# victorca25/traiNNer

Measured on AMD Instinct MI355X. Metric: HR images/sec (G+D step), ESRGAN x4 128->512, higher is better.
Workload: dtype f32 (bf16x3)

## Files before the change

### trainner_amd/csrc/conv_epilogue.h

```cpp
#pragma once
#include "conv_body.h"

namespace {

template <int MODE, int TW, int NT, int MT, bool COH, int DEPTH = 1, bool NOISE = true, int BIAS_STEP = 1, class PixFn>
__device__ __forceinline__ void conv_epilogue_dpp_map(const ConvK a, f32x16 (&acc)[MT][NT], const int cb, const int n, const int ty0,
                                                      const int tx0, const int par, const int li, const int half,
                                                      const __amdgpu_buffer_rsrc_t y_rs, PixFn &&pixfn) {
    constexpr bool DG2 = (MODE == TNR_DGRAD_4x4_S2);
    constexpr int NC = NT * 32;
    const int py = par >> 1, px = par & 1;
    TNR_STAMP(2);
#ifdef TNR_PRIO_EPI
    __builtin_amdgcn_s_setprio(TNR_PRIO_EPI);
#endif
    const int qa = li >> 2, qb = li & 3;
    const bool b0 = (qb & 1) != 0, b1 = (qb & 2) != 0;
    auto quad_transpose = [&](float &v0, float &v1, float &v2, float &v3) {
        auto xchg = [&](float &x, float &y, bool sel, int which) {
            const float send = sel ? x : y;
            const int r_ = which == 1 ? __builtin_amdgcn_mov_dpp(__builtin_bit_cast(int, send), 0xB1, 0xF, 0xF, true)
                                      : __builtin_amdgcn_mov_dpp(__builtin_bit_cast(int, send), 0x4E, 0xF, 0xF, true);
            const float recv = __builtin_bit_cast(float, r_);
            x = sel ? recv : x;
            y = sel ? y : recv;
        };
        xchg(v0, v1, b0, 1);
        xchg(v2, v3, b0, 1);
        xchg(v0, v2, b1, 2);
        xchg(v1, v3, b1, 2);
    };
    TNR_STAMP(5);
    TNR_STAMP(6);
    TNR_STAMP(7);
#ifdef TNR_ABL_NOMASK
    const bool has_r1 = a.r1 != nullptr, has_r2 = a.r2 != nullptr, has_m = false;
#else
    const bool has_r1 = a.r1 != nullptr, has_r2 = a.r2 != nullptr, has_m = a.m != nullptr;
#endif
    const bool has_noise = NOISE && a.noise_pos != 0;
    const bool all_full = (a.Cout & 3) == 0;
    const float ns = a.act == TNR_ACT_LRELU ? a.slope : (a.act == TNR_ACT_RELU ? 0.f : 1.f);
    int co_n[NT];
    bool co_ok[NT];
    f32x4 bv[NT];
    float b1f[NT], msf[NT];
    bool use_r1[NT], use_m[NT];
#pragma unroll
    for (int nn = 0; nn < NT; ++nn) {
        const int co = cb * NC + nn * 32 + qa * 4;
        co_n[nn] = co;
        co_ok[nn] = co < a.Cout;
        bv[nn] = f32x4{0.f, 0.f, 0.f, 0.f};
        if (a.bias != nullptr && co_ok[nn]) {
            if constexpr (BIAS_STEP != 1) {
#pragma unroll
                for (int k = 0; k < 4; ++k)
                    if (co + k < a.Cout) bv[nn][k] = a.bias[(co + k) * BIAS_STEP];
            } else if (co + 4 <= a.Cout) {
                bv[nn] = *reinterpret_cast<const f32x4 *>(a.bias + co);
            } else {
#pragma unroll
                for (int k = 0; k < 4; ++k)
                    if (co + k < a.Cout) bv[nn][k] = a.bias[co + k];
            }
        }
        use_r1[nn] = has_r1 && co < a.r1_ch;
        use_m[nn] = has_m && co >= a.m_lo && co < a.m_hi;
        b1f[nn] = use_r1[nn] ? a.beta1 : 0.f;
        msf[nn] = use_m[nn] ? a.m_slope : 1.f;
    }
    constexpr int UNITS = MT * 4;
    constexpr int AHEAD = DEPTH < UNITS ? DEPTH : UNITS, SETS = AHEAD + 1 < UNITS ? AHEAD + 1 : UNITS;
    bool ok[SETS];
    size_t pixi[SETS];
    f32x4 q1[SETS][NT], q2[SETS][NT], qm[SETS][NT];
    auto prep = [&](int u, int set) {
        const int mi = u >> 2, q = u & 3;
        int rr, cc;
        pixfn(mi, 8 * q + 4 * half + qb, rr, cc);
        const int sy = ty0 + rr, sx = tx0 + cc;
        ok[set] = sy < a.th_space && sx < a.tw_space;
        const int oy = DG2 ? 2 * sy + py : sy;
        const int ox = DG2 ? 2 * sx + px : sx;
        const size_t pix = ((size_t)n * a.Ho + oy) * a.Wo + ox;
        pixi[set] = pix;
        const f32x4 zero = {0.f, 0.f, 0.f, 0.f}, one = {1.f, 1.f, 1.f, 1.f};
#pragma unroll
        for (int nn = 0; nn < NT; ++nn) {
            const bool okc = ok[set] && co_ok[nn];
            if (has_r1) {
// ... 6 lines not shown
            }
            if (has_m) {
                qm[set][nn] = one;
                if (okc && use_m[nn]) qm[set][nn] = *reinterpret_cast<const f32x4 *>(a.m + pix * a.m_ct + a.m_co + co_n[nn]);
            }
        }
    };
    auto finish = [&](int u, int set) {
        const int mi = u >> 2, q = u & 3;
#pragma unroll
        for (int nn = 0; nn < NT; ++nn) {
            float v0 = acc[mi][nn][4 * q + 0], v1 = acc[mi][nn][4 * q + 1], v2 = acc[mi][nn][4 * q + 2], v3 = acc[mi][nn][4 * q + 3];
            quad_transpose(v0, v1, v2, v3);
            f32x4 v = f32x4{v0, v1, v2, v3} + bv[nn];
#pragma unroll
            for (int e = 0; e < 4; ++e) v[e] = __builtin_fmaf(ns, __builtin_fminf(v[e], 0.f), __builtin_fmaxf(v[e], 0.f)) * a.alpha;
            if (has_r1) v += b1f[nn] * q1[set][nn];
            if (has_noise) {
                const f32x4 nm = tnr_gauss_mult4(((unsigned)pixi[set] + a.noise_pix0) * (unsigned)(a.Cout >> 2) + (unsigned)(co_n[nn] >> 2),
                                                 a.noise_k0, a.noise_k1, a.noise_sigma);
                if (a.noise_pos == 1) v *= nm;
                if (has_r2) v = v * a.alpha2 + q2[set][nn];
                if (a.noise_pos != 1) v *= nm;
            } else if (has_r2) {
                v = v * a.alpha2 + q2[set][nn];
            }
            if (has_m) {
#pragma unroll
                for (int e = 0; e < 4; ++e) v[e] *= (qm[set][nn][e] > 0.f ? 1.f : msf[nn]);
            }
            if (!(ok[set] && co_ok[nn])) continue;
            const int co = co_n[nn];
#ifdef TNR_ABL_NOEPISTORE
            if (v[0] == 1.2345e30f) a.y[0] = v[1] + v[2] + v[3];
            continue;
#endif
            if (COH) {
                __builtin_amdgcn_raw_buffer_store_b128(__builtin_bit_cast(tnr_u32x4, v), y_rs,
                                                       (int)((unsigned)(pixi[set] * a.y_ct + a.y_co + co) * 4u), 0, TNR_COH_STORE_AUX);
            } else {
                float *yp = a.y + pixi[set] * a.y_ct + a.y_co + co;
                if (all_full) {
                    *reinterpret_cast<f32x4 *>(yp) = v;
                } else {
#pragma unroll
                    for (int e = 0; e < 4; ++e)
                        if (co + e < a.Cout) yp[e] = v[e];
                }
            }
        }
    };
#pragma unroll
    for (int u = 0; u < AHEAD; ++u) prep(u, u % SETS);
#pragma unroll
    for (int u = 0; u < UNITS; ++u) {
        if (u + AHEAD < UNITS) prep(u + AHEAD, (u + AHEAD) % SETS);
        finish(u, u % SETS);
    }
}

template <int MODE, int TW, int NT, int MT, bool COH, int DEPTH = 1, bool NOISE = true, int BIAS_STEP = 1>
__device__ __forceinline__ void conv_epilogue_dpp(const ConvK a, f32x16 (&acc)[MT][NT], const int cb, const int n, const int ty0,
                                                  const int tx0, const int par, const int wave, const int li, const int half,
                                                  const __amdgpu_buffer_rsrc_t y_rs) {
    conv_epilogue_dpp_map<MODE, TW, NT, MT, COH, DEPTH, NOISE, BIAS_STEP>(a, acc, cb, n, ty0, tx0, par, li, half, y_rs,
                                                                [&](int mi, int row, int &rr, int &cc) __attribute__((always_inline)) {
                                                                    const int p = (wave * MT + mi) * 32 + row;
                                                                    rr = p / TW;
                                                                    cc = p - rr * TW;
                                                                });
}

}
```

### trainner_amd/csrc/conv_sweep.hip

```cpp
#include <stddef.h>
#include <string.h>
#include <type_traits>
#include <utility>
#include "conv_body.h"
#include "conv_epilogue.h"
#include "conv_handoff.h"

namespace {

constexpr int SW_TH = 8, SW_TW = 32, SW_HT = SW_TH + 2, SW_WT = SW_TW + 2;
constexpr int SW_ROW = TNR_X3_ROW;
constexpr int SW_A_ROWS = SW_HT * SW_WT;
constexpr int SW_A_ALLOC_ROWS = 384;
constexpr int SW_A_FLOATS = SW_A_ALLOC_ROWS * SW_ROW;
constexpr int SW_UNIT_FLOATS = 32 * SW_ROW;
constexpr int SW_SLOT_UNITS = 9;
constexpr int SW_SLOT_FLOATS = SW_SLOT_UNITS * SW_UNIT_FLOATS;
constexpr int SW_RING = 3;
constexpr size_t SW_LDS_BYTES = (size_t)(2 * SW_A_FLOATS + SW_RING * SW_SLOT_FLOATS) * sizeof(float);
constexpr int SW_NPASS = 9, SW_NSTAGE = 5, SW_NTILE = 6;
constexpr int SW_A_IT = (SW_A_ROWS * 4 + 511) / 512;
constexpr int SW_B_PIECES = (SW_SLOT_UNITS * 3 + 7) / 8;
static_assert(SW_LDS_BYTES <= 160 * 1024, "one sweep workgroup per CU");

// ... 1083 lines not shown
        src = a.wp + (((size_t)par * 4 + tap) * a.KoutP + cb * 64 + j * 32 + r) * a.KinP + 16 * ck + 8 * h;
    } else {
        const int ck = rest % a.nck;
        rest /= a.nck;
        const int pp = rest & 3, cb = rest >> 2;
        src = a.wp + ((size_t)tap * a.KoutP + cb * 64 + j * 32 + r) * (4 * a.KinP) + pp * a.KinP + 16 * ck + 8 * h;
    }
    const f32x4 q0 = *reinterpret_cast<const f32x4 *>(src), q1 = *reinterpret_cast<const f32x4 *>(src + 4);
    tnr_bf16x8 pl[3];
    tnr_split_bf16x3(q0, q1, pl);
    float *dst = a.out + (size_t)unit * SW_UNIT_FLOATS + (h * 32 + r) * 4;
#pragma unroll
    for (int k = 0; k < 3; ++k) *reinterpret_cast<tnr_bf16x8 *>(dst + k * 256) = pl[k];
}

template <bool AMP, class Item, class BFetch>
__device__ __forceinline__ void tap4_chunk(f32x16 (&acc)[2][2], const float *sa, const int (&aaddr)[2][4], Item &&item_step,
                                           tnr_bf16x8 (&fbr)[S2_RING][3], BFetch &&b_fetch) {
    constexpr int TA[6] = {0, 2, 1, 0, 1, 0}, TB[6] = {2, 0, 1, 1, 0, 0};
    tnr_bf16x8 fa[2][2][3];
    auto read_a = [&](auto tc, int m, int sp) __attribute__((always_inline)) {
        constexpr int t = decltype(tc)::value;
        fa[t & 1][m][sp] = *reinterpret_cast<const tnr_bf16x8 *>(sa + aaddr[m][t] + 8 * sp);
    };
#pragma unroll
    for (int k = 0; k < (AMP ? 2 : 6); ++k) read_a(std::integral_constant<int, 0>{}, AMP ? k : k / 3, AMP ? 0 : k % 3);
    sw_static_for<0, S2_NU>([&](auto uc) __attribute__((always_inline)) {
        constexpr int u = decltype(uc)::value, t = u >> 1, jj = u & 1;
        constexpr bool NEXT_TAP = jj == 1 && t + 1 < S2_TAPS;
        constexpr int ITEM = u - (S2_NU - 6);
        __builtin_amdgcn_sched_barrier(0);
        if constexpr (AMP) {
            sw_static_for<0, 2>([&](auto mc) __attribute__((always_inline)) {
                constexpr int m = decltype(mc)::value;
                acc[m][jj] = __builtin_amdgcn_mfma_f32_32x32x16_bf16(fa[t & 1][m][0], fbr[u % S2_RING][0], acc[m][jj], 0, 0, 0);
                if constexpr (m == 0) b_fetch(std::integral_constant<int, (u + 3) % S2_RING>{}, 0);
                if constexpr (NEXT_TAP) read_a(std::integral_constant<int, (t + 1 < S2_TAPS ? t + 1 : t)>{}, m, 0);
                if constexpr (m == 1 && ITEM >= 0) item_step(std::integral_constant<int, (ITEM >= 0 ? ITEM : 0)>{}, std::integral_constant<int, -1>{});
                __builtin_amdgcn_sched_barrier(0);
            });
        } else {
            sw_static_for<0, 12>([&](auto ic) __attribute__((always_inline)) {
                constexpr int i = decltype(ic)::value, p = i / 2, m = i % 2;
                acc[m][jj] = __builtin_amdgcn_mfma_f32_32x32x16_bf16(fa[t & 1][m][TA[p]], fbr[u % S2_RING][TB[p]], acc[m][jj], 0, 0, 0);
                if constexpr (i < 3) b_fetch(std::integral_constant<int, (u + 3) % S2_RING>{}, i);
                if constexpr (NEXT_TAP && i >= 3 && i < 9) read_a(std::integral_constant<int, (t + 1 < S2_TAPS ? t + 1 : t)>{}, (i - 3) / 3, (i - 3) % 3);
                if constexpr (ITEM >= 0 && i >= 4 && i < 9) item_step(std::integral_constant<int, (ITEM >= 0 ? ITEM : 0)>{}, std::integral_constant<int, (i >= 4 && i < 9 ? i - 4 : 0)>{});
                __builtin_amdgcn_sched_barrier(0);
            });
        }
    });
}

template <int MODE, bool AMP>
__global__ void __launch_bounds__(256, 2) conv_s2_d4_kernel(const S2K c) {
    constexpr bool DG = MODE == TNR_DGRAD_4x4_S2;
    constexpr int HT = DG ? SW_HT : SW_TH + 1, WT = DG ? SW_WT : SW_TW + 1, ROWS = HT * WT;
    constexpr int A_IT = (ROWS * 4 + 255) / 256;
    static_assert(A_IT <= 6 && A_IT * 256 <= SW_A_ALLOC_ROWS * 4, "staging plan");
    extern __shared__ __attribute__((aligned(16))) float smem[];
    float *s_a = smem;
    const int tid = threadIdx.x;
    const int wave = __builtin_amdgcn_readfirstlane(tid >> 6), lane = tid & 63, li = lane & 31, half = lane >> 5;
    const ConvK &a = c.a;
    const __amdgpu_buffer_rsrc_t x_rs =
        __builtin_amdgcn_make_buffer_rsrc(const_cast<float *>(a.x), 0, (int)((unsigned)a.N * a.H * a.W * a.x_ct * 4u), 0x00020000);
    const __amdgpu_buffer_rsrc_t w_rs = __builtin_amdgcn_make_buffer_rsrc(const_cast<float *>(c.wq), 0, c.wq_bytes, 0x00020000);
    const __amdgpu_buffer_rsrc_t y_rs =
        __builtin_amdgcn_make_buffer_rsrc(a.y, 0, (int)((unsigned)a.N * a.Ho * a.Wo * a.y_ct * 4u), 0x00020000);
    const int nchunks = DG ? c.nck : 4 * c.nck;

    for (int tile = blockIdx.x; tile < c.tiles; tile += gridDim.x) {
        int rest = tile;
        const int cb = rest % c.ncb;
        rest /= c.ncb;
        int par = 0;
        if constexpr (DG) {
            par = rest & 3;
            rest >>= 2;
        }
        const int tx = rest % c.tiles_x;
        rest /= c.tiles_x;
        const int ty = rest % c.tiles_y, n = rest / c.tiles_y;
        const int ty0 = ty * SW_TH, tx0 = tx * SW_TW;
        const int py = par >> 1, px = par & 1;
        int aaddr[2][4];
#pragma unroll
        for (int m = 0; m < 2; ++m)
#pragma unroll
            for (int t = 0; t < 4; ++t) {
                const int pos_y = DG ? 1 + py - (t >> 1) : (t >> 1), pos_x = DG ? 1 + px - (t & 1) : (t & 1);
                const int pp = (2 * wave + m + pos_y) * WT + li + pos_x;
                aaddr[m][t] = pp * SW_ROW + 4 * (half ^ ((pp >> TNR_X3_SWZ) & 1));
            }
        int in_off[A_IT], a_dst[A_IT];
        auto plan = [&](int pp) __attribute__((always_inline)) {
#pragma unroll
            for (int it = 0; it < A_IT; ++it) {
                const int i = tid + it * 256, row = i >> 2, q = i & 3;
                const int hr = row / WT, hc = row - hr * WT;
                const int Y = DG ? ty0 + hr - 1 : 2 * (ty0 + hr) - 1 + (pp >> 1), X = DG ? tx0 + hc - 1 : 2 * (tx0 + hc) - 1 + (pp & 1);
                const bool in = (row < ROWS) & (Y >= 0) & (Y < a.H) & (X >= 0) & (X < a.W);
                in_off[it] = in ? (((n * a.H + Y) * a.W + X) * a.x_ct + a.x_co + q * 4) : -1;
                a_dst[it] = row * SW_ROW + 4 * ((q >> 1) ^ ((row >> TNR_X3_SWZ) & 1)) + 2 * (q & 1);
            }
        };
        plan(0);
// ... 34 lines not shown
        for (int m = 0; m < 2; ++m)
#pragma unroll
            for (int j = 0; j < 2; ++j)
#pragma unroll
                for (int r = 0; r < 16; ++r) acc[m][j][r] = 0.f;

        a_load(0, true);
        __syncthreads();
        tnr_bf16x8 fbr[S2_RING][3];
        int bq = (DG ? (par * c.ncb + cb) * c.nck : cb * 4 * c.nck) * S2_NU;
        auto b_fetch = [&](auto rc, int sp) __attribute__((always_inline)) {
            constexpr int r = decltype(rc)::value;
            if constexpr (AMP) {
                fbr[r][0] = __builtin_bit_cast(tnr_bf16x8, __builtin_amdgcn_raw_buffer_load_b128(w_rs, lane * 16, bq * 3072, 0));
                ++bq;
            } else {
                fbr[r][sp] = __builtin_bit_cast(tnr_bf16x8, __builtin_amdgcn_raw_buffer_load_b128(w_rs, lane * 16, (bq * 3 + sp) * 1024, 0));
                if (sp == 2) ++bq;
            }
        };
        sw_static_for<0, 3>([&](auto rc) __attribute__((always_inline)) {
#pragma unroll
            for (int sp = 0; sp < (AMP ? 1 : 3); ++sp) b_fetch(rc, sp);
        });
        sw_static_for<0, 6>([&](auto ic) __attribute__((always_inline)) {
            if constexpr (AMP) item_step_buf(ic, std::integral_constant<int, -1>{}, 0);
            else sw_static_for<0, 5>([&](auto kc) __attribute__((always_inline)) { item_step_buf(ic, kc, 0); });
        });
        bool has_next = false;
        int e = 0;
        auto item_step = [&](auto ic, auto kc) __attribute__((always_inline)) {
            if (has_next) item_step_buf(ic, kc, (e + 1) & 1);
        };
#pragma unroll 1
        for (int ck = 0; ck < nchunks; ++ck) {
            asm volatile("s_waitcnt lgkmcnt(0)\n\ts_barrier" ::: "memory");
            has_next = ck + 1 < nchunks;
            int ch_next = 16 * (ck + 1);
            if constexpr (!DG) {
                const int nx = ck + 1, ppn = nx / c.nck;
                ch_next = 16 * (nx - ppn * c.nck);
                if (has_next && ppn != ck / c.nck) plan(ppn);
            }
            a_load(ch_next, has_next);
            tap4_chunk<AMP>(acc, s_a + (e & 1) * SW_A_FLOATS, aaddr, item_step, fbr, b_fetch);
            ++e;
        }
        f32x16 t2[2][2];
#pragma unroll
        for (int m = 0; m < 2; ++m) {
            t2[m][0] = acc[m][0];
            t2[m][1] = acc[m][1];
        }
        conv_epilogue_dpp<MODE, SW_TW, 2, 2, false, 1>(a, t2, cb, n, ty0, tx0, par, wave, li, half, y_rs);
    }
}

bool s2_ok(const tnr_conv_desc *d) {
    if (d->mode != TNR_CONV_4x4_S2 && d->mode != TNR_DGRAD_4x4_S2) return false;
    const bool dg = d->mode == TNR_DGRAD_4x4_S2;
    const int tw = dg ? d->W : d->Wo, th = dg ? d->H : d->Ho;
    return (d->mma == TNR_MMA_BF16X3 || d->mma == TNR_MMA_BF16) && d->pad_mode == 0 && d->shuffle == 0 && (d->Cout % 64) == 0 && d->KoutP == d->Cout &&
           d->Cin == d->KinP && (d->Cin % 16) == 0 && d->Cin >= 32 && tw >= 32 && th >= 8 &&
           (dg ? (d->Ho == 2 * d->H && d->Wo == 2 * d->W) : (d->H == 2 * d->Ho && d->W == 2 * d->Wo)) &&
           buffers_addressable(*d) &&
           (int64_t)(d->Cout / 64) * (d->Cin / 16) * 4 * S2_NU * SW_UNIT_FLOATS * (int64_t)sizeof(float) < (1LL << 31);
}

bool d4_ok(const tnr_conv_desc *d) {
    if (d->shuffle != 0 && !(d->shuffle == 2 && (d->Cout % 256) == 0 && d->r1.ptr == nullptr && d->r2.ptr == nullptr && d->m.ptr == nullptr &&
                             d->noise_pos == 0 && d->pad_mode == 0 && (d->y.ctot % 4) == 0 &&
                             (int64_t)d->N * d->H * d->W * 4 * d->y.ctot < (1LL << 30)))
        return false;
    return d->mode == TNR_CONV_3x3 && (d->mma == TNR_MMA_BF16X3 || d->mma == TNR_MMA_BF16) && (d->pad_mode == 0 || (d->pad_mode == 1 && d->H >= 2 && d->W >= 2)) &&
           (d->Cout % 64) == 0 && d->KoutP == d->Cout &&
           d->Cin == d->KinP && (d->Cin % 16) == 0 && d->Cin >= 32 && d->Ho == d->H && d->Wo == d->W && d->W >= 32 && d->H >= 8 &&
           buffers_addressable(*d) &&
           (int64_t)(d->Cout / 64) * (d->Cin / 16) * 18 * SW_UNIT_FLOATS * (int64_t)sizeof(float) < (1LL << 31);
}

bool sweep_pattern(const tnr_conv_desc *st, int n, const char **why) {
    auto no = [&](const char *w) { if (why) *why = w; return false; };
    if (st == nullptr || (n != SW_NSTAGE && n != SW4_NSTAGE)) return no("not 5 (or 4) stages");
    if (n == SW4_NSTAGE && st[0].mma != TNR_MMA_BF16X3) return no("the four-stage form exists in bf16x3 only");
    const tnr_conv_desc &d0 = st[0];
    if (d0.Cin < 32 || (d0.Cin % 16) != 0) return no("block input channels must be a multiple of 16, >= 32");
    for (int i = 0; i < n; ++i) {
        const tnr_conv_desc &d = st[i];
        if (d.mode != TNR_CONV_3x3 || (d.mma != TNR_MMA_BF16X3 && d.mma != TNR_MMA_BF16) || d.mma != d0.mma || d.pad_mode != 0)
            return no("stage is not a zero-padded 3x3 in bf16x3 (or all stages with bf16 operands)");
        if (d.N != d0.N || d.H != d0.H || d.W != d0.W || d.Ho != d0.H || d.Wo != d0.W) return no("pixel grids differ");
        if (d.x.ptr != d0.x.ptr || d.x.ctot != d0.x.ctot || d.x.coff != d0.x.coff) return no("stages read different buffers");
        if (d.Cin != d0.Cin + 32 * i || d.KinP != d.Cin) return no("input channels do not grow by 32 per stage");
        if (d.Cout != (i < 4 ? 32 : 64) || d.KoutP != d.Cout) return no("output channels are not 32, 32, 32, 32, 64");
        if (i < 4 && (d.y.ptr != d0.x.ptr || d.y.ctot != d0.x.ctot || d.y.coff != d0.x.coff + d.Cin)) return no("stage output is not the next channel group");
        if (!views_aligned(d)) return no("x / y / r1 / r2 / mask views must be 4-channel aligned");
        if (d.noise_pos < 0 || d.noise_pos > 2 || (i < 4 && d.noise_pos != 0)) return no("the noise multiplier belongs to the last stage");
        if (!buffers_addressable(d)) return no("buffer above 4 GiB");
        if (!d.x.ptr || !d.y.ptr || !d.wp) return no("null pointer");
    }
    const tnr_conv_desc &dl = st[n - 1];
    if (n == SW_NSTAGE && dl.y.ptr == d0.x.ptr && dl.y.coff < d0.x.coff + dl.Cin && dl.y.coff + dl.Cout > d0.x.coff) return no("last stage overwrites its own input");
    return true;
}

int sweep_form() {
    static const int form = [] {
// ... 120 lines not shown
        k.tiles_x = c.tiles_x; k.tiles_y = c.tiles_y; k.ncb = d->KoutP / 32;
    }
    const int per_round = (cus / c.tpi) * c.tpi;
    const int grid = c.tiles < per_round ? c.tiles : per_round;
    const int form = sweep_form();
    if (n == SW4_NSTAGE) {
        TNR_REQUIRE(form == 5, "conv_sweep: four stages run in the direct four-wave form only");
        hipLaunchKernelGGL((conv_sweep4_kernel<true, false, SwPlan4>), dim3((unsigned)grid), dim3(256), S4D_LDS_BYTES, (hipStream_t)stream, c);
        return tnr_check_launch("conv_sweep");
    }
    if (stages[0].mma == TNR_MMA_BF16) {
        TNR_REQUIRE(form == 5, "conv_sweep: bf16 operands (use_amp) run in the direct four-wave form only");
        hipLaunchKernelGGL((conv_sweep4_kernel<true, true>), dim3((unsigned)grid), dim3(256), S4D_LDS_BYTES, (hipStream_t)stream, c);
        return tnr_check_launch("conv_sweep");
    }
    if (form == 8) hipLaunchKernelGGL(conv_sweep_kernel, dim3((unsigned)grid), dim3(512), SW_LDS_BYTES, (hipStream_t)stream, c);
    else if (form == 4) hipLaunchKernelGGL(conv_sweep4_kernel<false>, dim3((unsigned)grid), dim3(256), SW_LDS_BYTES, (hipStream_t)stream, c);
    else hipLaunchKernelGGL(conv_sweep4_kernel<true>, dim3((unsigned)grid), dim3(256), S4D_LDS_BYTES, (hipStream_t)stream, c);
    return tnr_check_launch("conv_sweep");
}

extern "C" int64_t tnr_conv_wq_bytes(const tnr_conv_desc *d) {
    if (d != nullptr && s2_ok(d)) return (int64_t)(d->Cout / 64) * (d->Cin / 16) * 4 * S2_NU * SW_UNIT_FLOATS * (int64_t)sizeof(float);
    if (d == nullptr || !d4_ok(d)) return 0;
    return (int64_t)(d->Cout / 64) * (d->Cin / 16) * 18 * SW_UNIT_FLOATS * (int64_t)sizeof(float);
}

extern "C" int tnr_conv_wq_pack(const tnr_conv_desc *d, void *image, int64_t image_bytes, void *stream) {
    if (d != nullptr && image != nullptr && d->wp != nullptr && s2_ok(d)) {
        S2PackK a;
        a.wp = d->wp; a.KinP = d->KinP; a.KoutP = d->KoutP; a.nck = d->Cin / 16; a.ncb = d->Cout / 64;
        a.dgrad = d->mode == TNR_DGRAD_4x4_S2;
        a.units = a.ncb * 4 * a.nck * S2_NU;
        TNR_REQUIRE((int64_t)a.units * SW_UNIT_FLOATS * (int64_t)sizeof(float) <= image_bytes, "conv_wq_pack: image buffer too small");
        a.out = static_cast<float *>(image);
        hipLaunchKernelGGL(s2_pack_kernel, dim3((unsigned)tnr_cdiv(a.units * 64, 256)), dim3(256), 0, (hipStream_t)stream, a);
        return tnr_check_launch("conv_wq_pack (four-tap form)");
    }
    TNR_REQUIRE(d != nullptr && image != nullptr && d->wp != nullptr && d4_ok(d), "conv_wq_pack: the launch cannot use a pre-split weight stream");
    D4PackK a;
    a.wp = d->wp; a.KinP = d->KinP; a.KoutP = d->KoutP; a.nck = d->Cin / 16; a.ncb = d->Cout / 64;
    a.units = a.ncb * a.nck * 18;
    a.shuffle = d->shuffle;
    TNR_REQUIRE((int64_t)a.units * SW_UNIT_FLOATS * (int64_t)sizeof(float) <= image_bytes, "conv_wq_pack: image buffer too small");
    a.out = static_cast<float *>(image);
    hipLaunchKernelGGL(d4_pack_kernel, dim3((unsigned)tnr_cdiv(a.units * 64, 256)), dim3(256), 0, (hipStream_t)stream, a);
    return tnr_check_launch("conv_wq_pack");
}

int tnr_launch_conv_s2_d4(const tnr_conv_desc *d, void *stream) {
    if (!s2_ok(d) || d->wq == nullptr || d->wq_bytes < tnr_conv_wq_bytes(d) || d->noise_pos != 0) return 1;
    static int cus = 0;
    if (const int rc = tnr_kernel_setup(&cus, "conv_s2_d4", {{conv_s2_d4_kernel<TNR_CONV_4x4_S2, false>, S4D_LDS_BYTES}, {conv_s2_d4_kernel<TNR_CONV_4x4_S2, true>, S4D_LDS_BYTES},
                                                             {conv_s2_d4_kernel<TNR_DGRAD_4x4_S2, false>, S4D_LDS_BYTES}, {conv_s2_d4_kernel<TNR_DGRAD_4x4_S2, true>, S4D_LDS_BYTES}}))
        return rc;
    const bool dg = d->mode == TNR_DGRAD_4x4_S2;
    S2K c;
    if (!stream_k_from_desc(c, *d, tnr_conv_wq_bytes(d), SW_TW, SW_TH, dg ? 4 : 1)) return 1;
    const unsigned grid = (unsigned)(c.tiles < 2 * cus ? c.tiles : 2 * cus);
    const bool amp = d->mma == TNR_MMA_BF16;
    if (dg) {
        if (amp) hipLaunchKernelGGL((conv_s2_d4_kernel<TNR_DGRAD_4x4_S2, true>), dim3(grid), dim3(256), S4D_LDS_BYTES, (hipStream_t)stream, c);
        else hipLaunchKernelGGL((conv_s2_d4_kernel<TNR_DGRAD_4x4_S2, false>), dim3(grid), dim3(256), S4D_LDS_BYTES, (hipStream_t)stream, c);
    } else {
        if (amp) hipLaunchKernelGGL((conv_s2_d4_kernel<TNR_CONV_4x4_S2, true>), dim3(grid), dim3(256), S4D_LDS_BYTES, (hipStream_t)stream, c);
        else hipLaunchKernelGGL((conv_s2_d4_kernel<TNR_CONV_4x4_S2, false>), dim3(grid), dim3(256), S4D_LDS_BYTES, (hipStream_t)stream, c);
    }
    return tnr_check_launch("conv_s2_d4");
}

int tnr_launch_conv3x3_d4(const tnr_conv_desc *d, void *stream) {
    if (!d4_ok(d) || d->wq == nullptr || d->wq_bytes < tnr_conv_wq_bytes(d) || d->noise_pos < 0 || d->noise_pos > 2) return 1;
    static int occ = [] { const char *e = getenv("TNR_D4_OCC"); return e ? atoi(e) : 2; }();
    static int cus = 0;
    if (const int rc = tnr_kernel_setup(&cus, "conv3x3_d4", {{conv3x3_d4_kernel<1>, S4D_LDS_BYTES}, {conv3x3_d4_kernel<2>, S4D_LDS_BYTES}, {conv3x3_d4_kernel<2, true>, S4D_LDS_BYTES},
                                                             {conv3x3_d4_kernel<2, false, true>, S4D_LDS_BYTES}, {conv3x3_d4_kernel<2, true, true>, S4D_LDS_BYTES}}))
        return rc;
    D4K c;
    if (!stream_k_from_desc(c, *d, tnr_conv_wq_bytes(d), SW_TW, SW_TH, 1)) return 1;
    const int slots = cus * (occ == 1 ? 1 : 2);
    const int grid = c.tiles < slots ? c.tiles : slots;
    if (d->shuffle == 2) {
        const unsigned g2 = (unsigned)(c.tiles < 2 * cus ? c.tiles : 2 * cus);
        if (d->mma == TNR_MMA_BF16) hipLaunchKernelGGL((conv3x3_d4_kernel<2, true, true>), dim3(g2), dim3(256), S4D_LDS_BYTES, (hipStream_t)stream, c);
        else hipLaunchKernelGGL((conv3x3_d4_kernel<2, false, true>), dim3(g2), dim3(256), S4D_LDS_BYTES, (hipStream_t)stream, c);
        return tnr_check_launch("conv3x3_d4 (pixel-shuffle store)");
    }
    if (d->mma == TNR_MMA_BF16) hipLaunchKernelGGL((conv3x3_d4_kernel<2, true>), dim3((unsigned)(c.tiles < 2 * cus ? c.tiles : 2 * cus)), dim3(256), S4D_LDS_BYTES, (hipStream_t)stream, c);
    else if (occ == 1) hipLaunchKernelGGL(conv3x3_d4_kernel<1>, dim3((unsigned)grid), dim3(256), S4D_LDS_BYTES, (hipStream_t)stream, c);
    else hipLaunchKernelGGL(conv3x3_d4_kernel<2>, dim3((unsigned)grid), dim3(256), S4D_LDS_BYTES, (hipStream_t)stream, c);
    return tnr_check_launch("conv3x3_d4");
}
```

### trainner_amd/csrc/conv_wino.hip

```cpp
#include <stddef.h>
#include <stdlib.h>
#include <type_traits>
#include <utility>
#include "conv_body.h"
#include "conv_epilogue.h"

namespace {

constexpr int WN_T = 16;
constexpr int WN_PT = WN_T / 2;
constexpr int WN_NP = WN_PT * WN_PT;
constexpr int WN_RAW_W = WN_T + 2;
constexpr int WN_RAW_PIX = WN_RAW_W * WN_RAW_W;
constexpr int WN_RAW_STRIDE = 24;
constexpr int WN_RAW_FLOATS = WN_RAW_PIX * WN_RAW_STRIDE;
constexpr int WN_ROW = TNR_X3_ROW;
constexpr int WN_VH_ROWS = 8 * WN_NP;
constexpr int WN_VH_FLOATS = WN_VH_ROWS * WN_ROW;
constexpr size_t WN_LDS_BYTES = (size_t)(2 * WN_VH_FLOATS + 2 * WN_RAW_FLOATS) * sizeof(float);
constexpr int WN_UNIT_FLOATS = 32 * WN_ROW;
constexpr int WN_STAGE_ITEMS = WN_RAW_PIX * 4;
constexpr int WN_STAGE_IT = (WN_STAGE_ITEMS / 2 + 255) / 256;
static_assert(WN_LDS_BYTES <= 160 * 1024, "one Winograd workgroup per CU");
static_assert(8 * 4 * 16 * 64 * sizeof(float) <= WN_LDS_BYTES, "the inverse transform's exchange fits the LDS");
// ... 14 lines not shown
struct WinoK {
    ConvK a;
    const float *wq;
    int wq_bytes;
    int nck;
    int tiles_x, tiles_y, ncb, tiles;
};

struct WinoPackK {
    const float *wp;
    int KinP, KoutP, nck, ncb, units;
    float *out;
};

__global__ void __launch_bounds__(256) wino_pack_kernel(const WinoPackK a) {
    const int g = blockIdx.x * 256 + threadIdx.x;
    const int unit = g >> 6, r = (g >> 1) & 31, oh = g & 1;
    if (unit >= a.units) return;
    const int j = unit & 3;
    int rest = unit >> 2;
    const int ck = rest % a.nck;
    rest /= a.nck;
    const int i = rest & 3, nt = (rest >> 2) & 1, cb = rest >> 3;
    const int co = cb * 64 + nt * 32 + r;
    const double G[4][3] = {{1.0, 0.0, 0.0}, {0.5, 0.5, 0.5}, {0.5, -0.5, 0.5}, {0.0, 0.0, 1.0}};
    f32x4 q[2];
#pragma unroll
    for (int e = 0; e < 8; ++e) {
        const int ch = 16 * ck + 8 * oh + e;
        double u = 0.0;
#pragma unroll
        for (int ky = 0; ky < 3; ++ky)
#pragma unroll
            for (int kx = 0; kx < 3; ++kx)
                u += G[i][ky] * G[j][kx] * (double)a.wp[((size_t)(ky * 3 + kx) * a.KoutP + co) * a.KinP + ch];
        q[e >> 2][e & 3] = (float)u;
    }
    tnr_bf16x8 pl[3];
    tnr_split_bf16x3(q[0], q[1], pl);
    float *dst = a.out + (size_t)unit * WN_UNIT_FLOATS + (oh * 32 + r) * 4;
#pragma unroll
    for (int k = 0; k < 3; ++k) *reinterpret_cast<tnr_bf16x8 *>(dst + k * 256) = pl[k];
}

template <int B, class F, int... I>
__device__ __forceinline__ void wn_static_for_seq(F &f, std::integer_sequence<int, I...>) {
    (f(std::integral_constant<int, B + I>{}), ...);
}
template <int B, int E, class F>
__device__ __forceinline__ void wn_static_for(F &&f) {
    wn_static_for_seq<B>(f, std::make_integer_sequence<int, (E > B ? E - B : 0)>{});
}

__global__ void __launch_bounds__(512, 2) conv3x3_wino_kernel(const WinoK c) {
    extern __shared__ __attribute__((aligned(16))) float smem[];
    float *s_v = smem;
    float *s_raw = smem + 2 * WN_VH_FLOATS;
    const int tid = threadIdx.x;
    const int wave = __builtin_amdgcn_readfirstlane(tid >> 6), lane = tid & 63, li = lane & 31, half = lane >> 5;
    const int wil = wave & 1, wn = (wave >> 1) & 1, wh = wave >> 2;
    const int wi = 2 * wh + wil;
    const int tt = tid & 255;
    const ConvK &a = c.a;
    const __amdgpu_buffer_rsrc_t x_rs =
        __builtin_amdgcn_make_buffer_rsrc(const_cast<float *>(a.x), 0, (int)((unsigned)a.N * a.H * a.W * a.x_ct * 4u), 0x00020000);
    const __amdgpu_buffer_rsrc_t w_rs = __builtin_amdgcn_make_buffer_rsrc(const_cast<float *>(c.wq), 0, c.wq_bytes, 0x00020000);
    const __amdgpu_buffer_rsrc_t y_rs =
        __builtin_amdgcn_make_buffer_rsrc(a.y, 0, (int)((unsigned)a.N * a.Ho * a.Wo * a.y_ct * 4u), 0x00020000);
    float *s_vh = s_v + wh * WN_VH_FLOATS;

    const int tp = tt >> 2, tq = tt & 3;
    const int tpy = tp >> 3, tpx = tp & 7;
    const int raw_off = ((2 * tpy + wh) * WN_RAW_W + 2 * tpx) * WN_RAW_STRIDE + 4 * tq;
    static_assert(TNR_X3_SWZ < 4, "the swizzle bit must not depend on the transform position or the M-tile");
    const int v_dst0 = tp * WN_ROW + 4 * ((tq >> 1) ^ ((tp >> TNR_X3_SWZ) & 1)) + 2 * (tq & 1);
    const int a_src0 = (wil * 4 * WN_NP + li) * WN_ROW + 4 * (half ^ ((li >> TNR_X3_SWZ) & 1));
    constexpr int XL_STRIDE = WN_NP * WN_ROW;

#ifdef WN_TIMELINE
    unsigned long long tl[16] = {0, 0, 0, 0, 0, 0, 0, 0, 0, 0, 0, 0, 0, 0, 0, 0};
    const unsigned long long tl_begin = __builtin_amdgcn_s_memtime();
#endif
    for (int tile = blockIdx.x; tile < c.tiles; tile += gridDim.x) {
        const int cb = tile % c.ncb;
        int rest = tile / c.ncb;
        const int tx = rest % c.tiles_x;
        rest /= c.tiles_x;
        const int ty = rest % c.tiles_y, n = rest / c.tiles_y;
        const int ty0 = ty * WN_T, tx0 = tx * WN_T;
        int in_off[WN_STAGE_IT], r_dst[WN_STAGE_IT];
#pragma unroll
        for (int it = 0; it < WN_STAGE_IT; ++it) {
            const int il = tt + it * 256;
            const int i = wh * (WN_STAGE_ITEMS / 2) + il, pix = i >> 2, q = i & 3;
            const int pr = pix / WN_RAW_W, pc = pix - pr * WN_RAW_W;
            int Y = ty0 + pr - 1, X = tx0 + pc - 1;
            if (a.reflect) {
                Y = Y == -1 ? 1 : (Y == a.H ? a.H - 2 : Y);
                X = X == -1 ? 1 : (X == a.W ? a.W - 2 : X);
            }
            const bool mine = il < WN_STAGE_ITEMS / 2;
            const bool in = mine & (Y >= 0) & (Y < a.H) & (X >= 0) & (X < a.W);
            in_off[it] = in ? (((n * a.H + Y) * a.W + X) * a.x_ct + a.x_co + q * 4) : -1;
            r_dst[it] = mine ? pix * WN_RAW_STRIDE + 4 * q : -1;
        }
        f32x4 rin[WN_STAGE_IT];
// ... 183 lines not shown
        for (int ck = 0; ck < c.nck; ++ck) {
            WN_T(t0);
#ifndef WN_X_NORAW
            if (ck >= 1 && ck + 1 < c.nck) raw_store((ck + 1) & 1);
#endif
#if !defined(WN_X_NOB) && defined(WN_B_EARLY)
            b_fetch(ck, std::integral_constant<int, 0>{});
#elif defined(WN_X_NOB)
            if (ck == 0) { b_fetch(0, std::integral_constant<int, 0>{}); b_fetch(0, std::integral_constant<int, 2>{}); }
#endif
            { WN_T(ts); WN_ADD(8, ts); WN_ADD(13, t0); }
#ifndef WN_X_NOT
            transform(ck & 1);
#endif
#if !defined(WN_X_NOB) && !defined(WN_B_EARLY)
            b_fetch(ck, std::integral_constant<int, 0>{});
#endif
            WN_T(t1);
            __syncthreads();
            WN_T(t2);
#ifndef WN_X_NOB
            b_fetch(ck, std::integral_constant<int, 2>{});
#endif
#ifndef WN_X_NORAW
            raw_load(16 * (ck + 2), ck + 2 < c.nck);
#endif
#ifndef WN_X_NOM
            multiply();
#endif
            WN_T(t3);
            __syncthreads();
            WN_T(t4);
            WN_ADD(0, t1 - t0); WN_ADD(1, t2 - t1); WN_ADD(2, t3 - t2); WN_ADD(3, t4 - t3); WN_ADD(7, 1ull);
        }
        if (wh == 0) __syncthreads();
        WN_T(t_loop1);
        WN_ADD(4, t_loop1 - t_loop0);

#ifdef WN_X_NOEPI
        if (a.alpha == 1.2345e30f)
#endif
        {
        {
            float *xch = smem + wave * (4 * 16 * 64);
#pragma unroll
            for (int l = 0; l < 2; ++l)
#pragma unroll
                for (int m = 0; m < 2; ++m) {
                    const f32x16 rr = l == 0 ? (acc[0][m] + acc[1][m]) + acc[2][m] : (acc[1][m] - acc[2][m]) - acc[3][m];
#pragma unroll
                    for (int r = 0; r < 16; ++r) xch[((l * 2 + m) * 16 + r) * 64 + lane] = rr[r];
                }
        }
        __syncthreads();
        f32x16 keep[2][1];
        {
            const int k = wil, m = wh;
            auto slot = [&](int ip, int l) __attribute__((always_inline)) {
                return smem + (((ip >> 1) * 4 + wn * 2 + (ip & 1)) * 4 + l * 2 + m) * (16 * 64) + lane;
            };
#pragma unroll
            for (int l = 0; l < 2; ++l) {
                const float *p0 = slot(k, l), *p1 = slot(k + 1, l), *p2 = slot(k + 2, l);
#pragma unroll
                for (int r = 0; r < 16; ++r) {
                    const float x0 = p0[r * 64], x1 = p1[r * 64], x2 = p2[r * 64];
                    keep[l][0][r] = k == 0 ? (x0 + x1) + x2 : (x0 - x1) - x2;
                }
            }
        }
        conv_epilogue_dpp_map<TNR_CONV_3x3, WN_T, 1, 2, false, 1>(a, keep, cb * 2 + wn, n, ty0, tx0, 0, li, half, y_rs,
                                                                  [&](int mi, int row, int &rr, int &cc) __attribute__((always_inline)) {
                                                                      const int p = 32 * wh + row;
                                                                      rr = 2 * (p >> 3) + wil;
                                                                      cc = 2 * (p & 7) + mi;
                                                                  });
        }
    }
#ifdef WN_TIMELINE
    if (lane == 0 && (wave & 3) == 0) {
        tl[5] = __builtin_amdgcn_s_memtime() - tl_begin;
        for (int i = 0; i < 16; ++i) atomicAdd(&wn_tl[wh][i], tl[i]);
    }
#endif
}

constexpr int W16_STAGE_IT = (WN_STAGE_ITEMS / 2 + 511) / 512;

__global__ void __launch_bounds__(1024, 4) conv3x3_wino16_kernel(const WinoK c) {
    extern __shared__ __attribute__((aligned(16))) float smem[];
    float *s_v = smem;
    float *s_raw = smem + 2 * WN_VH_FLOATS;
    const int tid = threadIdx.x;
    const int wave = __builtin_amdgcn_readfirstlane(tid >> 6), lane = tid & 63, li = lane & 31, half = lane >> 5;
    const int wh = (wave >> 2) & 1, role = (wave & 3) | ((wave >> 3) << 2);
    const int wil = role & 1, wn = (role >> 1) & 1, wjp = role >> 2;
    const int wi = 2 * wh + wil;
    const int tt = role * 64 + lane;
    const ConvK &a = c.a;
    const __amdgpu_buffer_rsrc_t x_rs =
        __builtin_amdgcn_make_buffer_rsrc(const_cast<float *>(a.x), 0, (int)((unsigned)a.N * a.H * a.W * a.x_ct * 4u), 0x00020000);
    const __amdgpu_buffer_rsrc_t w_rs = __builtin_amdgcn_make_buffer_rsrc(const_cast<float *>(c.wq), 0, c.wq_bytes, 0x00020000);
    const __amdgpu_buffer_rsrc_t y_rs =
        __builtin_amdgcn_make_buffer_rsrc(a.y, 0, (int)((unsigned)a.N * a.Ho * a.Wo * a.y_ct * 4u), 0x00020000);
    float *s_vh = s_v + wh * WN_VH_FLOATS;

    const int tp = (tt >> 2) & 63, tq = tt & 3, rs = tt >> 8;
    const int tpy = tp >> 3, tpx = tp & 7;
    const int it_ = 2 * wh + rs;
    const int pa = it_ == 0 ? 0 : (it_ == 2 ? 2 : 1), pb = it_ == 0 ? 2 : (it_ == 1 ? 2 : (it_ == 2 ? 1 : 3));
    const bool plus = it_ == 1;
    const int raw_a = ((2 * tpy + pa) * WN_RAW_W + 2 * tpx) * WN_RAW_STRIDE + 4 * tq;
    const int raw_b = ((2 * tpy + pb) * WN_RAW_W + 2 * tpx) * WN_RAW_STRIDE + 4 * tq;
    static_assert(TNR_X3_SWZ < 4, "the swizzle bit must not depend on the transform position or the M-tile");
    const int v_dst0 = (rs * 4 * WN_NP + tp) * WN_ROW + 4 * ((tq >> 1) ^ ((tp >> TNR_X3_SWZ) & 1)) + 2 * (tq & 1);
    const int a_src0 = ((wil * 4 + 2 * wjp) * WN_NP + li) * WN_ROW + 4 * (half ^ ((li >> TNR_X3_SWZ) & 1));
    constexpr int XL_STRIDE = WN_NP * WN_ROW;

    for (int tile = blockIdx.x; tile < c.tiles; tile += gridDim.x) {
        const int cb = tile % c.ncb;
        int rest = tile / c.ncb;
        const int tx = rest % c.tiles_x;
        rest /= c.tiles_x;
        const int ty = rest % c.tiles_y, n = rest / c.tiles_y;
        const int ty0 = ty * WN_T, tx0 = tx * WN_T;
        int in_off[W16_STAGE_IT], r_dst[W16_STAGE_IT];
#pragma unroll
        for (int it = 0; it < W16_STAGE_IT; ++it) {
            const int il = tt + it * 512;
            const int i = wh * (WN_STAGE_ITEMS / 2) + il, pix = i >> 2, q = i & 3;
// ... 159 lines not shown
            for (int r = 0; r < 16; ++r) {
                const float x0 = p0[r * 64], x1 = p1[r * 64], x2 = p2[r * 64];
                keep[0][0][r] = k == 0 ? (x0 + x1) + x2 : (x0 - x1) - x2;
            }
        }
        conv_epilogue_dpp_map<TNR_CONV_3x3, WN_T, 1, 1, false, 1>(a, keep, cb * 2 + wn, n, ty0, tx0, 0, li, half, y_rs,
                                                                  [&](int, int row, int &rr, int &cc) __attribute__((always_inline)) {
                                                                      const int p = 32 * wh + row;
                                                                      rr = 2 * (p >> 3) + wil;
                                                                      cc = 2 * (p & 7) + wjp;
                                                                  });
    }
}

bool wino_ok(const tnr_conv_desc *d) {
    return d->mode == TNR_CONV_3x3 && d->mma == TNR_MMA_BF16X3 && (d->pad_mode == 0 || (d->pad_mode == 1 && d->H >= 2 && d->W >= 2)) &&
           (d->Cout % 64) == 0 && d->KoutP == d->Cout && d->Cin == d->KinP && (d->Cin % 16) == 0 && d->Cin >= 32 && d->Ho == d->H &&
           d->Wo == d->W && d->W >= 8 && d->H >= 8 && buffers_addressable(*d) &&
           (int64_t)(d->Cout / 64) * (d->Cin / 16) * 32 * WN_UNIT_FLOATS * (int64_t)sizeof(float) < (1LL << 31);
}

}

#ifdef WN_TIMELINE
extern "C" int tnr_debug_wino_timeline(unsigned long long *out16, int reset) {
    if (out16 != nullptr && hipMemcpyFromSymbol(out16, HIP_SYMBOL(wn_tl), sizeof(wn_tl)) != hipSuccess) return TNR_ELAUNCH;
    if (reset) {
        unsigned long long z[32] = {0};
        if (hipMemcpyToSymbol(HIP_SYMBOL(wn_tl), z, sizeof(z)) != hipSuccess) return TNR_ELAUNCH;
    }
    return TNR_OK;
}
#endif

extern "C" int64_t tnr_conv_wino_bytes(const tnr_conv_desc *d) {
    if (d == nullptr || !wino_ok(d)) return 0;
    return (int64_t)(d->Cout / 64) * (d->Cin / 16) * 32 * WN_UNIT_FLOATS * (int64_t)sizeof(float);
}

extern "C" int tnr_conv_wino_pack(const tnr_conv_desc *d, void *image, int64_t image_bytes, void *stream) {
    TNR_REQUIRE(d != nullptr && image != nullptr && d->wp != nullptr && wino_ok(d), "conv_wino_pack: the launch cannot run in the Winograd form");
    WinoPackK a;
    a.wp = d->wp; a.KinP = d->KinP; a.KoutP = d->KoutP; a.nck = d->Cin / 16; a.ncb = d->Cout / 64;
    a.units = a.ncb * a.nck * 32;
    TNR_REQUIRE((int64_t)a.units * WN_UNIT_FLOATS * (int64_t)sizeof(float) <= image_bytes, "conv_wino_pack: image buffer too small");
    a.out = static_cast<float *>(image);
    hipLaunchKernelGGL(wino_pack_kernel, dim3((unsigned)tnr_cdiv(a.units * 64, 256)), dim3(256), 0, (hipStream_t)stream, a);
    return tnr_check_launch("conv_wino_pack");
}

int tnr_launch_conv3x3_wino(const tnr_conv_desc *d, void *stream) {
    if (!wino_ok(d) || d->wq == nullptr || d->wq_bytes < tnr_conv_wino_bytes(d) || d->noise_pos < 0 || d->noise_pos > 2) return 1;
    static int cus = 0;
    if (const int rc = tnr_kernel_setup(&cus, "conv3x3_wino", {{conv3x3_wino_kernel, WN_LDS_BYTES}, {conv3x3_wino16_kernel, WN_LDS_BYTES}})) return rc;
    WinoK c;
    if (!stream_k_from_desc(c, *d, tnr_conv_wino_bytes(d), WN_T, WN_T, 1)) return 1;
    const int grid = c.tiles < cus ? c.tiles : cus;
    static const bool w16 = [] { const char *e = getenv("TNR_WINO_WAVES"); return e != nullptr && atoi(e) == 16; }();
    if (w16) {
        hipLaunchKernelGGL(conv3x3_wino16_kernel, dim3((unsigned)grid), dim3(1024), WN_LDS_BYTES, (hipStream_t)stream, c);
        return tnr_check_launch("conv3x3_wino16");
    }
    hipLaunchKernelGGL(conv3x3_wino_kernel, dim3((unsigned)grid), dim3(512), WN_LDS_BYTES, (hipStream_t)stream, c);
    return tnr_check_launch("conv3x3_wino");
}
```

Baseline: 76.15.

## Prefetch epilogue residual/mask loads ahead of the final barrier and row transform

Adds a 'between' hook and a KINDS template mask to the DPP conv epilogue so the residual and mask loads can be issued before the last __syncthreads and the Winograd output row transform, with a prefetch depth of 8. The Winograd 3x3 kernel gains an AHEAD variant that is used whenever residual or mask inputs exist. The stride-2 dgrad kernel gains a mask-only variant with depth 8 and only mask loads compiled in. The aim is to hide global load latency in the epilogue behind the barrier and the LDS transform, at the cost of more registers held across the barrier and extra kernel instantiations.

```diff
diff --git a/trainner_amd/csrc/conv_epilogue.h b/trainner_amd/csrc/conv_epilogue.h
--- a/trainner_amd/csrc/conv_epilogue.h
+++ b/trainner_amd/csrc/conv_epilogue.h
@@ -3,10 +3,24 @@
 
 namespace {
 
-template <int MODE, int TW, int NT, int MT, bool COH, int DEPTH = 1, bool NOISE = true, int BIAS_STEP = 1, class PixFn>
+constexpr int EPI_R1 = 1, EPI_R2 = 2, EPI_M = 4, EPI_ALL = 7;
+struct EpiNoBetween {
+    __device__ __forceinline__ void operator()() const {}
+};
+
+inline bool tnr_epi_ahead() {
+    const char *e = getenv("TNR_EPI_AHEAD");
+    return !(e != nullptr && e[0] == '0');
+}
+inline int tnr_epi_kinds(const tnr_conv_desc &d) {
+    return (d.r1.ptr != nullptr ? EPI_R1 : 0) | (d.r2.ptr != nullptr ? EPI_R2 : 0) | (d.m.ptr != nullptr ? EPI_M : 0);
+}
+
+template <int MODE, int TW, int NT, int MT, bool COH, int DEPTH = 1, bool NOISE = true, int BIAS_STEP = 1, int KINDS = EPI_ALL, class PixFn,
+          class Between = EpiNoBetween>
 __device__ __forceinline__ void conv_epilogue_dpp_map(const ConvK a, f32x16 (&acc)[MT][NT], const int cb, const int n, const int ty0,
                                                       const int tx0, const int par, const int li, const int half,
-                                                      const __amdgpu_buffer_rsrc_t y_rs, PixFn &&pixfn) {
+                                                      const __amdgpu_buffer_rsrc_t y_rs, PixFn &&pixfn, Between &&between = Between{}) {
     constexpr bool DG2 = (MODE == TNR_DGRAD_4x4_S2);
     constexpr int NC = NT * 32;
     const int py = par >> 1, px = par & 1;
@@ -36,7 +50,8 @@
 #ifdef TNR_ABL_NOMASK
     const bool has_r1 = a.r1 != nullptr, has_r2 = a.r2 != nullptr, has_m = false;
 #else
-    const bool has_r1 = a.r1 != nullptr, has_r2 = a.r2 != nullptr, has_m = a.m != nullptr;
+    const bool has_r1 = (KINDS & EPI_R1) != 0 && a.r1 != nullptr, has_r2 = (KINDS & EPI_R2) != 0 && a.r2 != nullptr,
+               has_m = (KINDS & EPI_M) != 0 && a.m != nullptr;
 #endif
     const bool has_noise = NOISE && a.noise_pos != 0;
     const bool all_full = (a.Cout & 3) == 0;
@@ -149,6 +164,7 @@
     };
 #pragma unroll
     for (int u = 0; u < AHEAD; ++u) prep(u, u % SETS);
+    between();
 #pragma unroll
     for (int u = 0; u < UNITS; ++u) {
         if (u + AHEAD < UNITS) prep(u + AHEAD, (u + AHEAD) % SETS);
@@ -156,11 +172,11 @@
     }
 }
 
-template <int MODE, int TW, int NT, int MT, bool COH, int DEPTH = 1, bool NOISE = true, int BIAS_STEP = 1>
+template <int MODE, int TW, int NT, int MT, bool COH, int DEPTH = 1, bool NOISE = true, int BIAS_STEP = 1, int KINDS = EPI_ALL>
 __device__ __forceinline__ void conv_epilogue_dpp(const ConvK a, f32x16 (&acc)[MT][NT], const int cb, const int n, const int ty0,
                                                   const int tx0, const int par, const int wave, const int li, const int half,
                                                   const __amdgpu_buffer_rsrc_t y_rs) {
-    conv_epilogue_dpp_map<MODE, TW, NT, MT, COH, DEPTH, NOISE, BIAS_STEP>(a, acc, cb, n, ty0, tx0, par, li, half, y_rs,
+    conv_epilogue_dpp_map<MODE, TW, NT, MT, COH, DEPTH, NOISE, BIAS_STEP, KINDS>(a, acc, cb, n, ty0, tx0, par, li, half, y_rs,
                                                                 [&](int mi, int row, int &rr, int &cc) __attribute__((always_inline)) {
                                                                     const int p = (wave * MT + mi) * 32 + row;
                                                                     rr = p / TW;
diff --git a/trainner_amd/csrc/conv_sweep.hip b/trainner_amd/csrc/conv_sweep.hip
--- a/trainner_amd/csrc/conv_sweep.hip
+++ b/trainner_amd/csrc/conv_sweep.hip
@@ -1159,7 +1159,7 @@
     });
 }
 
-template <int MODE, bool AMP>
+template <int MODE, bool AMP, int KINDS = 0>
 __global__ void __launch_bounds__(256, 2) conv_s2_d4_kernel(const S2K c) {
     constexpr bool DG = MODE == TNR_DGRAD_4x4_S2;
     constexpr int HT = DG ? SW_HT : SW_TH + 1, WT = DG ? SW_WT : SW_TW + 1, ROWS = HT * WT;
@@ -1300,7 +1300,13 @@
             t2[m][0] = acc[m][0];
             t2[m][1] = acc[m][1];
         }
-        conv_epilogue_dpp<MODE, SW_TW, 2, 2, false, 1>(a, t2, cb, n, ty0, tx0, par, wave, li, half, y_rs);
+        if constexpr (KINDS != 0) {
+            int li_e = li, half_e = half;
+            asm volatile("" : "+v"(li_e), "+v"(half_e));
+            conv_epilogue_dpp<MODE, SW_TW, 2, 2, false, 8, true, 1, KINDS>(a, t2, cb, n, ty0, tx0, par, wave, li_e, half_e, y_rs);
+        } else {
+            conv_epilogue_dpp<MODE, SW_TW, 2, 2, false, 1>(a, t2, cb, n, ty0, tx0, par, wave, li, half, y_rs);
+        }
     }
 }
 
@@ -1527,13 +1533,19 @@
     if (!s2_ok(d) || d->wq == nullptr || d->wq_bytes < tnr_conv_wq_bytes(d) || d->noise_pos != 0) return 1;
     static int cus = 0;
     if (const int rc = tnr_kernel_setup(&cus, "conv_s2_d4", {{conv_s2_d4_kernel<TNR_CONV_4x4_S2, false>, S4D_LDS_BYTES}, {conv_s2_d4_kernel<TNR_CONV_4x4_S2, true>, S4D_LDS_BYTES},
-                                                             {conv_s2_d4_kernel<TNR_DGRAD_4x4_S2, false>, S4D_LDS_BYTES}, {conv_s2_d4_kernel<TNR_DGRAD_4x4_S2, true>, S4D_LDS_BYTES}}))
+                                                             {conv_s2_d4_kernel<TNR_DGRAD_4x4_S2, false>, S4D_LDS_BYTES}, {conv_s2_d4_kernel<TNR_DGRAD_4x4_S2, true>, S4D_LDS_BYTES},
+                                                             {conv_s2_d4_kernel<TNR_DGRAD_4x4_S2, false, EPI_M>, S4D_LDS_BYTES}, {conv_s2_d4_kernel<TNR_DGRAD_4x4_S2, true, EPI_M>, S4D_LDS_BYTES}}))
         return rc;
     const bool dg = d->mode == TNR_DGRAD_4x4_S2;
     S2K c;
     if (!stream_k_from_desc(c, *d, tnr_conv_wq_bytes(d), SW_TW, SW_TH, dg ? 4 : 1)) return 1;
     const unsigned grid = (unsigned)(c.tiles < 2 * cus ? c.tiles : 2 * cus);
     const bool amp = d->mma == TNR_MMA_BF16;
+    if (dg && tnr_epi_ahead() && tnr_epi_kinds(*d) == EPI_M) {
+        if (amp) hipLaunchKernelGGL((conv_s2_d4_kernel<TNR_DGRAD_4x4_S2, true, EPI_M>), dim3(grid), dim3(256), S4D_LDS_BYTES, (hipStream_t)stream, c);
+        else hipLaunchKernelGGL((conv_s2_d4_kernel<TNR_DGRAD_4x4_S2, false, EPI_M>), dim3(grid), dim3(256), S4D_LDS_BYTES, (hipStream_t)stream, c);
+        return tnr_check_launch("conv_s2_d4");
+    }
     if (dg) {
         if (amp) hipLaunchKernelGGL((conv_s2_d4_kernel<TNR_DGRAD_4x4_S2, true>), dim3(grid), dim3(256), S4D_LDS_BYTES, (hipStream_t)stream, c);
         else hipLaunchKernelGGL((conv_s2_d4_kernel<TNR_DGRAD_4x4_S2, false>), dim3(grid), dim3(256), S4D_LDS_BYTES, (hipStream_t)stream, c);
diff --git a/trainner_amd/csrc/conv_wino.hip b/trainner_amd/csrc/conv_wino.hip
--- a/trainner_amd/csrc/conv_wino.hip
+++ b/trainner_amd/csrc/conv_wino.hip
@@ -90,6 +90,7 @@
     wn_static_for_seq<B>(f, std::make_integer_sequence<int, (E > B ? E - B : 0)>{});
 }
 
+template <bool AHEAD = false>
 __global__ void __launch_bounds__(512, 2) conv3x3_wino_kernel(const WinoK c) {
     extern __shared__ __attribute__((aligned(16))) float smem[];
     float *s_v = smem;
@@ -379,9 +380,8 @@
                     for (int r = 0; r < 16; ++r) xch[((l * 2 + m) * 16 + r) * 64 + lane] = rr[r];
                 }
         }
-        __syncthreads();
         f32x16 keep[2][1];
-        {
+        auto row_step = [&]() __attribute__((always_inline)) {
             const int k = wil, m = wh;
             auto slot = [&](int ip, int l) __attribute__((always_inline)) {
                 return smem + (((ip >> 1) * 4 + wn * 2 + (ip & 1)) * 4 + l * 2 + m) * (16 * 64) + lane;
@@ -395,14 +395,31 @@
                     keep[l][0][r] = k == 0 ? (x0 + x1) + x2 : (x0 - x1) - x2;
                 }
             }
-        }
-        conv_epilogue_dpp_map<TNR_CONV_3x3, WN_T, 1, 2, false, 1>(a, keep, cb * 2 + wn, n, ty0, tx0, 0, li, half, y_rs,
-                                                                  [&](int mi, int row, int &rr, int &cc) __attribute__((always_inline)) {
-                                                                      const int p = 32 * wh + row;
-                                                                      rr = 2 * (p >> 3) + wil;
-                                                                      cc = 2 * (p & 7) + mi;
-                                                                  });
-        }
+        };
+        auto pixfn = [&](int mi, int row, int &rr, int &cc) __attribute__((always_inline)) {
+            const int p = 32 * wh + row;
+            rr = 2 * (p >> 3) + wil;
+            cc = 2 * (p & 7) + mi;
+        };
+        if constexpr (AHEAD) {
+            __builtin_amdgcn_sched_barrier(0);
+            conv_epilogue_dpp_map<TNR_CONV_3x3, WN_T, 1, 2, false, 8>(a, keep, cb * 2 + wn, n, ty0, tx0, 0, li, half, y_rs, pixfn,
+                                                                      [&]() __attribute__((always_inline)) {
+                                                                          __syncthreads();
+                                                                          row_step();
+                                                                      });
+        } else {
+            __syncthreads();
+            row_step();
+            conv_epilogue_dpp_map<TNR_CONV_3x3, WN_T, 1, 2, false, 1>(a, keep, cb * 2 + wn, n, ty0, tx0, 0, li, half, y_rs, pixfn);
+        }
+        }
+#ifdef WN_TIMELINE
+        __builtin_amdgcn_sched_barrier(0);
+        { WN_T(t_tail); WN_ADD(6, t_tail - t_loop1); WN_ADD(14, 1ull);
+          asm volatile("s_waitcnt vmcnt(0)" ::: "memory");
+          WN_T(t_ack); WN_ADD(15, t_ack - t_tail); }
+#endif
     }
 #ifdef WN_TIMELINE
     if (lane == 0 && (wave & 3) == 0) {
@@ -668,15 +685,17 @@
 int tnr_launch_conv3x3_wino(const tnr_conv_desc *d, void *stream) {
     if (!wino_ok(d) || d->wq == nullptr || d->wq_bytes < tnr_conv_wino_bytes(d) || d->noise_pos < 0 || d->noise_pos > 2) return 1;
     static int cus = 0;
-    if (const int rc = tnr_kernel_setup(&cus, "conv3x3_wino", {{conv3x3_wino_kernel, WN_LDS_BYTES}, {conv3x3_wino16_kernel, WN_LDS_BYTES}})) return rc;
+    if (const int rc = tnr_kernel_setup(&cus, "conv3x3_wino", {{conv3x3_wino_kernel<false>, WN_LDS_BYTES}, {conv3x3_wino_kernel<true>, WN_LDS_BYTES}, {conv3x3_wino16_kernel, WN_LDS_BYTES}})) return rc;
     WinoK c;
     if (!stream_k_from_desc(c, *d, tnr_conv_wino_bytes(d), WN_T, WN_T, 1)) return 1;
     const int grid = c.tiles < cus ? c.tiles : cus;
+    const bool ahead = tnr_epi_ahead() && tnr_epi_kinds(*d) != 0;
     static const bool w16 = [] { const char *e = getenv("TNR_WINO_WAVES"); return e != nullptr && atoi(e) == 16; }();
     if (w16) {
         hipLaunchKernelGGL(conv3x3_wino16_kernel, dim3((unsigned)grid), dim3(1024), WN_LDS_BYTES, (hipStream_t)stream, c);
         return tnr_check_launch("conv3x3_wino16");
     }
-    hipLaunchKernelGGL(conv3x3_wino_kernel, dim3((unsigned)grid), dim3(512), WN_LDS_BYTES, (hipStream_t)stream, c);
+    if (ahead) hipLaunchKernelGGL(conv3x3_wino_kernel<true>, dim3((unsigned)grid), dim3(512), WN_LDS_BYTES, (hipStream_t)stream, c);
+    else hipLaunchKernelGGL(conv3x3_wino_kernel<false>, dim3((unsigned)grid), dim3(512), WN_LDS_BYTES, (hipStream_t)stream, c);
     return tnr_check_launch("conv3x3_wino");
 }
```

After: 76.28, median of 2. Within noise of the previous version (+0.2%).
